# EllarBooher/Syzygy

Hardware: AMD Instinct MI355X
Metric: Mpixels/s deferred-lit+atmosphere (higher is better)
Workload: dtype f32

## Files before the change

### syzygy_amd/csrc/api_skyview.cpp

```cpp

#include <new>

#include "api_common.hpp"
#include "lut_state.hpp"

using namespace szg;

struct szg_skyview
{
    int device = 0;
    szg_skyview_desc desc{};
    DeviceBuffer<float> d_transmittance, d_skyview, d_multiscatter, d_aerialLuminance, d_aerialTransmittance;
    float aerialMaxDistance = 0.0f;
    mutable LutState luts;
    DeviceBuffer<unsigned> d_slutStatusAll;
    bool lutReuse = false;
    DeviceBuffer<unsigned> d_lutKey;
    DeviceBuffer<void> d_framePrep;
    DeviceBuffer<void> d_framePrepDraw;
};

static hipError_t ensure_tlut_status(szg_skyview* p, hipStream_t s)
{
    hipError_t e = hipSuccess;
// ... 89 lines not shown
    }
    return SZG_OK;
}

void szg_skyview_destroy(szg_skyview_t* p)
{
    if (p == nullptr)
    {
        return;
    }
    (void)hipSetDevice(p->device);
    delete p;
}

int szg_skyview_transmittance_lut(const szg_skyview_t* p, szg_image* out)
{
    if (p == nullptr || out == nullptr)
    {
        return fail(SZG_ERR_INVALID_ARGUMENT, "szg_skyview_transmittance_lut: NULL argument");
    }
    *out = make_image(p->d_transmittance, p->desc.transmittance_width, p->desc.transmittance_height, SZG_FORMAT_RGBA32_SFLOAT);
    p->luts.transmittance_exposed();
    return SZG_OK;
}

int szg_skyview_skyview_lut(const szg_skyview_t* p, szg_image* out)
{
    if (p == nullptr || out == nullptr)
    {
        return fail(SZG_ERR_INVALID_ARGUMENT, "szg_skyview_skyview_lut: NULL argument");
    }
    *out = make_image(p->d_skyview, p->desc.skyview_width, p->desc.skyview_height, SZG_FORMAT_RGBA32_SFLOAT);
    p->luts.skyview_exposed();
    return SZG_OK;
}

int szg_skyview_record_transmittance(szg_skyview_t* p, void* stream, uint32_t atmosphere_index,
                                     const szg_atmosphere_packed* d_atmospheres)
{
    if (p == nullptr || d_atmospheres == nullptr)
    {
        return fail(SZG_ERR_INVALID_ARGUMENT, "szg_skyview_record_transmittance: NULL argument");
    }
    DeviceGuard const guard(p->device);
    hipStream_t const s = static_cast<hipStream_t>(stream);
    const unsigned* dirty = nullptr;
    if (p->lutReuse)
    {
        SZG_HIP(szg::launch_lut_key(s, d_atmospheres, atmosphere_index, nullptr, 0u, p->d_lutKey, 0u, p->luts.forceTransmittance,
                                    p->d_transmittance, p->desc.transmittance_width, p->desc.transmittance_height));
        dirty = p->d_lutKey + 69;
    }
    SZG_HIP(szg::launch_transmittance(s, d_atmospheres, atmosphere_index, p->d_transmittance, p->desc.transmittance_width,
                                      p->desc.transmittance_height, dirty));
    p->luts.transmittance_recorded();
    return SZG_OK;
}

int szg_skyview_record_skyview_lut_rows(szg_skyview_t* p, void* stream, uint32_t atmosphere_index,
                                        const szg_atmosphere_packed* d_atmospheres, uint32_t view_camera_index,
                                        const szg_camera_packed* d_cameras, uint32_t row_begin, uint32_t row_end)
{
    if (p == nullptr || d_atmospheres == nullptr || d_cameras == nullptr)
    {
        return fail(SZG_ERR_INVALID_ARGUMENT, "szg_skyview_record_skyview_lut_rows: NULL argument");
    }
    if (row_begin > row_end || row_end > p->desc.skyview_height)
    {
        return fail(SZG_ERR_INVALID_ARGUMENT, "szg_skyview_record_skyview_lut_rows: rows [%u, %u) outside the %u-row LUT", row_begin,
                    row_end, p->desc.skyview_height);
    }
    DeviceGuard const guard(p->device);
    hipStream_t const s = static_cast<hipStream_t>(stream);
    bool const whole = LutState::whole(row_begin, row_end, p->desc.skyview_height);
    SZG_HIP(ensure_tlut_status(p, s));
    const unsigned* dirty = nullptr;
    if (p->lutReuse && whole)
    {
        SZG_HIP(szg::launch_lut_key(s, d_atmospheres, atmosphere_index, d_cameras, view_camera_index, p->d_lutKey, 1u, p->luts.forceSkyview,
                                    p->d_skyview, p->desc.skyview_width, p->desc.skyview_height));
        dirty = p->d_lutKey + 70;
    }
    SZG_HIP(szg::launch_frame_prep(s, d_atmospheres, atmosphere_index, p->desc.transmittance_width, p->desc.transmittance_height,
                                   p->d_framePrep));
    SZG_HIP(szg::launch_skyview(s, d_atmospheres, atmosphere_index, d_cameras, view_camera_index, p->d_transmittance,
                                p->desc.transmittance_width, p->desc.transmittance_height, p->d_skyview, p->desc.skyview_width,
                                p->desc.skyview_height, row_begin, row_end, dirty, p->d_framePrep));
    p->luts.skyview_rows_recorded(row_begin, row_end, p->desc.skyview_height);
    return SZG_OK;
}

int szg_skyview_lut_row_slice(const szg_skyview_t* p, uint32_t rank, uint32_t nranks, uint32_t* row_begin, uint32_t* row_end)
{
    if (p == nullptr || row_begin == nullptr || row_end == nullptr || nranks == 0u || rank >= nranks)
    {
        return fail(SZG_ERR_INVALID_ARGUMENT, "szg_skyview_lut_row_slice: NULL argument or rank outside [0, nranks)");
    }
    if (p->desc.skyview_height % nranks != 0u)
    {
        return fail(SZG_ERR_INVALID_ARGUMENT, "szg_skyview_lut_row_slice: %u LUT rows do not divide over %u ranks", p->desc.skyview_height,
                    nranks);
    }
    uint32_t const n = p->desc.skyview_height / nranks;
    *row_begin = rank * n;
    *row_end = (rank + 1u) * n;
    return SZG_OK;
}

int szg_skyview_allgather_lut_rows(szg_skyview_t* p, szg_rowtile_comm_t* comm, void* stream)
{
    if (p == nullptr || comm == nullptr)
    {
        return fail(SZG_ERR_INVALID_ARGUMENT, "szg_skyview_allgather_lut_rows: NULL argument");
    }
    int const nranks = szg_rowtile_comm_size(comm);
    if (nranks < 1 || p->desc.skyview_height % (uint32_t)nranks != 0u)
    {
        return fail(SZG_ERR_INVALID_ARGUMENT, "szg_skyview_allgather_lut_rows: %u LUT rows do not divide over %d ranks",
                    p->desc.skyview_height, nranks);
    }
    if (nranks > (int)szg::SLUT_STATUS_RANKS)
    {
        return fail(SZG_ERR_INVALID_ARGUMENT, "szg_skyview_allgather_lut_rows: more than %u ranks", szg::SLUT_STATUS_RANKS);
    }
    DeviceGuard const guard(p->device);
    hipStream_t const s = static_cast<hipStream_t>(stream);
    size_t const slice = (size_t)(p->desc.skyview_height / (uint32_t)nranks) * p->desc.skyview_width * 16u;
    unsigned const rank = (unsigned)szg_rowtile_comm_rank(comm);
    bool const known = p->luts.slice_status_known(rank, (uint32_t)nranks, p->desc.skyview_height);
    SZG_HIP(szg::launch_slut_status_stage(s, p->d_slutStatusAll, rank, p->d_skyview, p->desc.skyview_width,
                                          p->desc.skyview_height, known));
    int rc = szg_rowtile_allgather(comm, stream, p->d_skyview, slice);
    if (rc == SZG_OK)
    {
        rc = szg_rowtile_allgather(comm, stream, p->d_slutStatusAll, sizeof(unsigned));
    }
    if (rc == SZG_OK)
    {
        SZG_HIP(szg::launch_slut_status_reduce(s, p->d_slutStatusAll, (unsigned)nranks, p->d_skyview, p->desc.skyview_width,
                                               p->desc.skyview_height));
    }
    p->luts.rows_gathered(rc == SZG_OK);
    return rc;
}

int szg_skyview_record_skyview_lut(szg_skyview_t* p, void* stream, uint32_t atmosphere_index,
                                   const szg_atmosphere_packed* d_atmospheres, uint32_t view_camera_index,
                                   const szg_camera_packed* d_cameras)
{
    if (p == nullptr)
    {
        return fail(SZG_ERR_INVALID_ARGUMENT, "szg_skyview_record_skyview_lut: NULL argument");
    }
    return szg_skyview_record_skyview_lut_rows(p, stream, atmosphere_index, d_atmospheres, view_camera_index, d_cameras, 0u,
                                               p->desc.skyview_height);
}

static int record_composite(szg_skyview_t* p, void* stream, const szg_scene_texture* scene_texture, szg_rect draw_rect,
                            const szg_rowtile* tile, const szg_gbuffer* gbuffer, const szg_shadowmaps* shadow_maps,
                            uint32_t atmosphere_index, const szg_atmosphere_packed* d_atmospheres, uint32_t view_camera_index,
                            const szg_camera_packed* d_cameras, uint32_t sun_light_index,
                            const szg_directional_light_packed* d_lights, bool fast)
{
    if (p == nullptr || d_atmospheres == nullptr || d_cameras == nullptr || d_lights == nullptr)
    {
        return fail(SZG_ERR_INVALID_ARGUMENT, "szg_skyview_record_composite: NULL argument");
    }
    if (!check_rect(draw_rect, "szg_skyview_record_composite"))
    {
        return SZG_ERR_INVALID_ARGUMENT;
    }
    DeviceGuard const guard(p->device);
    if (draw_rect.width == 0u || draw_rect.height == 0u)
    {
        return SZG_OK;
    }
    szg::TileArgs t{};
    if (!resolve_tile(tile, draw_rect.height, t))
    {
        return SZG_ERR_INVALID_ARGUMENT;
    }
    if (!check_scene(scene_texture, draw_rect.width, t.local_rows, true) || !check_gbuffer(gbuffer, draw_rect.width, t.local_rows))
    {
        return SZG_ERR_INVALID_ARGUMENT;
    }
    szg::ShadowSlot sun{nullptr, 0u, 0u, 0u, 0u};
    if (shadow_maps != nullptr && shadow_maps->maps != nullptr && sun_light_index < shadow_maps->count &&
        shadow_maps->maps[sun_light_index].data != nullptr)
    {
        const szg_image& m = shadow_maps->maps[sun_light_index];
        if (!check_image(m, SZG_FORMAT_D32_SFLOAT, 1u, 1u, "shadow map"))
        {
            return SZG_ERR_INVALID_ARGUMENT;
        }
        sun = szg::ShadowSlot{static_cast<const float*>(m.data), m.width, m.height, m.pitch_bytes / 4u, 0u};
    }
    szg::AerialLut aerial{nullptr, SZG_AERIAL_W, SZG_AERIAL_H, SZG_AERIAL_D, 0.0f};
    if (fast)
    {
        if (!(p->aerialMaxDistance > 0.0f))
        {
            return fail(SZG_ERR_INVALID_ARGUMENT, "szg_skyview_record_composite_fast: no aerial LUT has been recorded");
        }
        aerial.luminance = p->d_aerialLuminance;
        aerial.maxDistance = p->aerialMaxDistance;
    }
    SZG_HIP(ensure_tlut_status(p, static_cast<hipStream_t>(stream)));
    SZG_HIP(ensure_slut_status(p, static_cast<hipStream_t>(stream)));
    SZG_HIP(szg::launch_frame_prep(static_cast<hipStream_t>(stream), d_atmospheres, atmosphere_index, p->desc.transmittance_width,
                                   p->desc.transmittance_height, p->d_framePrepDraw,
                                   sun.map != nullptr ? d_lights + sun_light_index : nullptr));
    SZG_HIP(szg::launch_composite(static_cast<hipStream_t>(stream), *scene_texture, draw_rect.width, draw_rect.height, t, *gbuffer,
                                  sun, d_atmospheres, atmosphere_index, d_cameras, view_camera_index, d_lights, sun_light_index,
                                  p->d_transmittance, p->desc.transmittance_width, p->desc.transmittance_height, p->d_skyview,
                                  p->desc.skyview_width, p->desc.skyview_height, aerial, p->d_framePrepDraw));
    return SZG_OK;
}

int szg_skyview_record_composite(szg_skyview_t* p, void* stream, const szg_scene_texture* scene_texture, szg_rect draw_rect,
                                 const szg_rowtile* tile, const szg_gbuffer* gbuffer, const szg_shadowmaps* shadow_maps,
                                 uint32_t atmosphere_index, const szg_atmosphere_packed* d_atmospheres,
                                 uint32_t view_camera_index, const szg_camera_packed* d_cameras, uint32_t sun_light_index,
                                 const szg_directional_light_packed* d_lights)
{
    return record_composite(p, stream, scene_texture, draw_rect, tile, gbuffer, shadow_maps, atmosphere_index, d_atmospheres,
                            view_camera_index, d_cameras, sun_light_index, d_lights, false);
}

int szg_skyview_record_composite_fast(szg_skyview_t* p, void* stream, const szg_scene_texture* scene_texture, szg_rect draw_rect,
                                      const szg_rowtile* tile, const szg_gbuffer* gbuffer, const szg_shadowmaps* shadow_maps,
                                      uint32_t atmosphere_index, const szg_atmosphere_packed* d_atmospheres,
                                      uint32_t view_camera_index, const szg_camera_packed* d_cameras, uint32_t sun_light_index,
                                      const szg_directional_light_packed* d_lights)
{
    return record_composite(p, stream, scene_texture, draw_rect, tile, gbuffer, shadow_maps, atmosphere_index, d_atmospheres,
                            view_camera_index, d_cameras, sun_light_index, d_lights, true);
}

int szg_skyview_record_multiscatter_lut(szg_skyview_t* p, void* stream, uint32_t atmosphere_index,
                                        const szg_atmosphere_packed* d_atmospheres)
{
    if (p == nullptr || d_atmospheres == nullptr)
    {
        return fail(SZG_ERR_INVALID_ARGUMENT, "szg_skyview_record_multiscatter_lut: NULL argument");
    }
    DeviceGuard const guard(p->device);
    SZG_HIP(ensure_tlut_status(p, static_cast<hipStream_t>(stream)));
    SZG_HIP(szg::launch_multiscatter(static_cast<hipStream_t>(stream), d_atmospheres, atmosphere_index, p->d_transmittance,
                                     p->desc.transmittance_width, p->desc.transmittance_height, p->d_multiscatter,
                                     SZG_MULTISCATTER_DIM));
    return SZG_OK;
}

int szg_skyview_multiscatter_lut(const szg_skyview_t* p, szg_image* out)
{
    if (p == nullptr || out == nullptr)
    {
        return fail(SZG_ERR_INVALID_ARGUMENT, "szg_skyview_multiscatter_lut: NULL argument");
    }
    *out = make_image(p->d_multiscatter, SZG_MULTISCATTER_DIM, SZG_MULTISCATTER_DIM, SZG_FORMAT_RGBA32_SFLOAT);
    return SZG_OK;
}

int szg_skyview_record_aerial_lut(szg_skyview_t* p, void* stream, uint32_t atmosphere_index,
                                  const szg_atmosphere_packed* d_atmospheres, uint32_t view_camera_index,
                                  const szg_camera_packed* d_cameras, float max_distance_mm)
{
    if (p == nullptr || d_atmospheres == nullptr || d_cameras == nullptr)
    {
        return fail(SZG_ERR_INVALID_ARGUMENT, "szg_skyview_record_aerial_lut: NULL argument");
    }
    if (!(max_distance_mm > 0.0f) || !(max_distance_mm < 1.0e6f))
    {
        return fail(SZG_ERR_INVALID_ARGUMENT, "szg_skyview_record_aerial_lut: max_distance_mm must be in (0, 1e6)");
    }
    DeviceGuard const guard(p->device);
    SZG_HIP(ensure_tlut_status(p, static_cast<hipStream_t>(stream)));
    SZG_HIP(szg::launch_aerial_lut(static_cast<hipStream_t>(stream), d_atmospheres, atmosphere_index, d_cameras, view_camera_index,
                                   p->d_transmittance, p->desc.transmittance_width, p->desc.transmittance_height,
                                   p->d_aerialLuminance, p->d_aerialTransmittance, SZG_AERIAL_W, SZG_AERIAL_H, SZG_AERIAL_D,
                                   max_distance_mm));
    p->aerialMaxDistance = max_distance_mm;
    return SZG_OK;
}

int szg_skyview_aerial_lut(const szg_skyview_t* p, szg_image* out_luminance, szg_image* out_transmittance)
{
    if (p == nullptr || out_luminance == nullptr || out_transmittance == nullptr)
    {
        return fail(SZG_ERR_INVALID_ARGUMENT, "szg_skyview_aerial_lut: NULL argument");
    }
    *out_luminance = make_image(p->d_aerialLuminance, SZG_AERIAL_W, SZG_AERIAL_H * SZG_AERIAL_D, SZG_FORMAT_RGBA32_SFLOAT);
    *out_transmittance = make_image(p->d_aerialTransmittance, SZG_AERIAL_W, SZG_AERIAL_H * SZG_AERIAL_D, SZG_FORMAT_RGBA32_SFLOAT);
    return SZG_OK;
// ... 16 lines not shown
```

### syzygy_amd/csrc/kernels_lut.hip

```cpp

#include "szg_device.hpp"
#include "szg_launch.hpp"

namespace szg
{
template <int CTRL> SZG_DEV float dpp(float v)
{
    return __builtin_bit_cast(float, __builtin_amdgcn_update_dpp(0, __builtin_bit_cast(int, v), CTRL, 0xF, 0xF, false));
}

constexpr int T_LANES = 8;
constexpr int T_STEPS = 500;

template <bool LEAN> SZG_DEV V3 transmittanceProduct(const Atm& a, V3 origin, V3 direction, float distance, float ndt, int sub)
{
    V3 T = splat(1.0f);
    float const rcp500 = rcpN(500.0f);
#pragma unroll 1
    for (int k = 0; k < (T_STEPS + T_LANES - 1) / T_LANES; k++)
    {
        int const i = k * T_LANES + sub;
        float const t = divRX<LEAN>(distance * ((float)i + 0.5f), 500.0f, rcp500);
        V3 const position = origin + t * direction;
        float const altitude = sqrtPX<LEAN>(dotT(position, position)) - a.planetRadius;
        Extinction const e = sampleExtinction<LEAN>(a, altitude);
        bool const valid = i < T_STEPS;
        float const fx = valid ? expX<LEAN>(ndt * e.extinction.x) : 1.0f;
        float const fy = valid ? expX<LEAN>(ndt * e.extinction.y) : 1.0f;
        float const fz = valid ? expX<LEAN>(ndt * e.extinction.z) : 1.0f;
        T.x = dpp<0x107>(T.x) * fx;
        T.y = dpp<0x107>(T.y) * fy;
        T.z = dpp<0x107>(T.z) * fz;
#pragma unroll
        for (int j = 1; j < T_LANES; j++)
        {
            T.x = dpp<0x111>(T.x) * fx;
            T.y = dpp<0x111>(T.y) * fy;
            T.z = dpp<0x111>(T.z) * fz;
        }
    }
    return T;
}

__global__ __launch_bounds__(256) void k_transmittance(const szg_atmosphere_packed* __restrict__ atmospheres,
                                                      unsigned atmosphereIndex, float4* __restrict__ lut, int W, int H,
                                                      const unsigned* __restrict__ dirty)
{
    if (dirty != nullptr && dirty[0] == 0u)
    {
        return;
    }
    int const sub = (int)(threadIdx.x & (unsigned)(T_LANES - 1));
    int const idRaw = (int)((blockIdx.x * 256u + threadIdx.x) / (unsigned)T_LANES);
    bool const inRangeTexel = idRaw < W * H;
    int const id = inRangeTexel ? idRaw : (W * H - 1);
    int const tx = id % W;
    int const ty = id / W;
    Atm const a = load_atm(atmospheres + atmosphereIndex);

    float const u = ((float)tx + 0.5f) / (float)W;
    float const v = ((float)ty + 0.5f) / (float)H;

    float const x_mu = (u - 0.5f / (float)W) / (1.0f - 1.0f / (float)W);
    float const x_radius = (v - 0.5f / (float)H) / (1.0f - 1.0f / (float)H);
    float const rho = a.H * x_radius;
    float const radius = sqrtf(rho * rho + a.Rp2);
    float const d_min = a.atmosphereRadius - radius;
    float const d_max = rho + a.H;
    float const d = (d_max - d_min) * x_mu + d_min;
    float mu = 1.0f;
    if (d != 0.0f)
    {
        mu = clampf((a.H * a.H - rho * rho - d * d) / (2.0f * radius * d), -1.0f, 1.0f);
    }

    V3 const origin = mk3(0.0f, radius, 0.0f);
    V3 const direction = mk3(sqrtf(1.0f - mu * mu), mu, 0.0f);

    float t0 = 0.0f, t1 = 0.0f;
    bool const hit = raySphere(origin, direction, a.atmosphereRadius, t0, t1);
    float const distance = hit ? t1 : 0.0f;
    float const dt = distance / 500.0f;
    float const ndt = -fabsf(dt);
    float const rmin2 = mu < 0.0f ? radius * radius * (1.0f - mu * mu) : radius * radius;
    bool const lean = waveAll(a.lean && rmin2 >= a.leanFloor2 && inRange(radius, 0x1p-30f, 0x1p30f) && inRange(distance, 0.0f, 0x1p30f));
    V3 const T = lean ? transmittanceProduct<true>(a, origin, direction, distance, ndt, sub)
                      : transmittanceProduct<false>(a, origin, direction, distance, ndt, sub);
    if (inRangeTexel && sub == T_LANES - 1)
    {
        float4 const texel = hit ? make_float4(T.x, T.y, T.z, 1.0f) : make_float4(1.0f, 1.0f, 1.0f, 1.0f);
        lut[id] = texel;
        if (!tlutTexelModerate(texel.x, texel.y, texel.z))
        {
            atomicOr(reinterpret_cast<unsigned*>(lut + (size_t)W * (size_t)H), 1u);
        }
    }
}

__global__ __launch_bounds__(256) void k_lut_range(float4* __restrict__ lut, unsigned n)
{
    unsigned const id = blockIdx.x * 256u + threadIdx.x;
    bool ok = true;
    if (id < n)
    {
        float4 const t = lut[id];
        ok = tlutTexelModerate(t.x, t.y, t.z);
    }
    if (!waveAll(ok) && (threadIdx.x & 63u) == 0u)
    {
        atomicOr(reinterpret_cast<unsigned*>(lut + n), 1u);
    }
}

__global__ __launch_bounds__(64) void k_frame_prep(const szg_atmosphere_packed* __restrict__ atmospheres, unsigned atmosphereIndex,
                                                   int tW, int tH, FramePrep* __restrict__ out,
                                                   const szg_directional_light_packed* __restrict__ sun)
{
    if (threadIdx.x != 0u)
    {
        return;
    }
    FramePrep f;
    f.a = load_atm(atmospheres + atmosphereIndex);
    f.fwidth = (float)tW;
    f.fheight = (float)tH;
    f.u_bias = 0.5f / (float)tW;
    f.u_scale = 1.0f - 1.0f / (float)tW;
    f.v_bias = 0.5f / (float)tH;
    f.v_scale = 1.0f - 1.0f / (float)tH;
    {
        auto vOf = [&](float x_radius) {
            float const t = SZG_CON(SZG_C_LUTMAP, x_radius, f.v_scale, f.v_bias);
            return SZG_CON(SZG_C_TEXCOORD, t, f.fheight, -0.5f);
        };
        float const rMax = sqrtf(f.a.innerCeil2) * (1.0f + 0x1p-16f);
        float const rhoMax = safeSqrt(rMax * rMax - f.a.Rp2);
        float const vLo = vOf(0.0f), vHi = vOf(rhoMax / f.a.H);
        bool const ok = f.a.lean && vLo >= 0.0f && floorf(vHi) + 1.0f <= f.fheight - 1.0f && vHi == vHi && tW >= 2 && tH >= 2 &&
                        (float)tW * (float)tH <= 0x1p24f;
        f.rowsInterior = ok ? 1u : 0u;
    }
#pragma unroll
    for (int k = 0; k < 16; k++)
    {
        f.sunShadow[k] = 0.0f;
    }
    if (sun != nullptr)
    {
        M4 toTex;
        float const t[16] = {0.5f, 0.0f, 0.0f, 0.0f, 0.0f, 0.5f, 0.0f, 0.0f, 0.0f, 0.0f, 1.0f, 0.0f, 0.5f, 0.5f, 0.0f, 1.0f};
#pragma unroll
        for (int k = 0; k < 16; k++)
        {
            toTex.m[k] = t[k];
        }
        M4 const sm = mul(toTex, mul(load_m4(sun->projection), load_m4(sun->view)));
#pragma unroll
        for (int k = 0; k < 16; k++)
        {
            f.sunShadow[k] = sm.m[k];
        }
    }
    *out = f;
}

__global__ __launch_bounds__(256, 4) void k_skyview(const szg_atmosphere_packed* __restrict__ atmospheres, unsigned atmosphereIndex,
                                                 const szg_camera_packed* __restrict__ cameras, unsigned cameraIndex,
                                                 const float4* __restrict__ tlut, int tW, int tH, float4* __restrict__ lut,
                                                 int W, int H, int rowBegin, int rowEnd, const unsigned* __restrict__ dirty,
                                                 const FramePrep* __restrict__ prep)
{
    if (dirty != nullptr && dirty[0] == 0u)
    {
        return;
    }
    unsigned const tid = threadIdx.x;
    unsigned const wave = tid >> 6, lane = tid & 63u;
    int const x = (int)(blockIdx.x * 32u + wave * 8u + (lane & 7u));
    int const y = rowBegin + (int)(blockIdx.y * 8u + (lane >> 3));
    if (x >= W || y >= rowEnd)
    {
        return;
    }
    Atm const a = load_atm(*prep);
    TLut const L = make_tlut(tlut, tW, tH, *prep);
    const szg_camera_packed* cam = cameras + cameraIndex;
    float const PI = 3.141592653589793f;

    float const u = ((float)x + 0.5f) / (float)W;
    float const v = ((float)y + 0.5f) / (float)H;

    V3 origin = mk3(cam->position[0], cam->position[1], cam->position[2]) / 1000000.0f;
    origin.y *= -1.0f;
    origin.y += a.planetRadius;

    float const radius = length(origin);
    float const sinHorizonZenith = a.planetRadius / radius;
    float const horizonZenith = PI - szg_asinf(sinHorizonZenith);
    float const cosineViewLightProjected = (u - 0.5f) * 2.0f;
    V2 const lightDirectionProjected = normalize(V2{-a.incidentDirectionSun.x, -a.incidentDirectionSun.z});
    float azimuthSun = szg_asinf(lightDirectionProjected.x);
    if (lightDirectionProjected.y < 0.0f)
    {
        azimuthSun = PI - azimuthSun;
    }
    float const azimuth = szg_acosf(clampf(cosineViewLightProjected, -1.0f, 1.0f)) + azimuthSun;
    float viewZenith;
    float const unnormalized_v = 2.0f * v - 1.0f;
    if (v < 0.5f)
    {
        float const angleFraction = 1.0f - unnormalized_v * unnormalized_v;
        viewZenith = angleFraction * horizonZenith;
    }
    else
    {
        float const angleFraction = unnormalized_v * unnormalized_v;
        viewZenith = (PI - horizonZenith) * angleFraction + horizonZenith;
    }
    float const elevation = -(viewZenith - PI / 2.0f);

    float const ce = szg_cosf(elevation);
    V3 const direction = normalize(mk3(szg_sinf(azimuth) * ce, szg_sinf(elevation), szg_cosf(azimuth) * ce));

    float const distance = raycastAtmosphere(a, origin, direction);
    V3 const luminance = scatteringIntegral(L, a, origin, direction, distance);
    lut[y * W + x] = make_float4(luminance.x, luminance.y, luminance.z, 1.0f);
    if (!slutTexelFinite(luminance.x, luminance.y, luminance.z))
    {
        atomicOr(reinterpret_cast<unsigned*>(lut + (size_t)W * (size_t)H), 1u);
    }
}

__global__ __launch_bounds__(256) void k_slut_check(float4* __restrict__ lut, unsigned n)
{
    unsigned const id = blockIdx.x * 256u + threadIdx.x;
    bool ok = true;
    if (id < n)
    {
        float4 const t = lut[id];
        ok = slutTexelFinite(t.x, t.y, t.z);
    }
    if (!waveAll(ok) && (threadIdx.x & 63u) == 0u)
    {
        atomicOr(reinterpret_cast<unsigned*>(lut + n), 1u);
    }
}

__global__ void k_slut_status_stage(unsigned* __restrict__ all, unsigned rank, const unsigned* __restrict__ status, unsigned known)
{
    if (threadIdx.x == 0u)
    {
        all[rank] = known != 0u ? status[0] : 1u;
    }
}
__global__ void k_slut_status_reduce(const unsigned* __restrict__ all, unsigned nranks, unsigned* __restrict__ status)
{
    if (threadIdx.x == 0u)
    {
        unsigned v = 0u;
        for (unsigned r = 0; r < nranks; r++)
        {
            v |= all[r];
        }
        status[0] = v;
    }
}

__global__ __launch_bounds__(256) void k_aerial_lut(const szg_atmosphere_packed* __restrict__ atmospheres, unsigned atmosphereIndex,
                                                    const szg_camera_packed* __restrict__ cameras, unsigned cameraIndex,
                                                    const float4* __restrict__ tlut, int tW, int tH, float4* __restrict__ luminance,
                                                    float4* __restrict__ transmittance, unsigned W, unsigned H, unsigned D,
                                                    float maxDistance)
{
    unsigned const id = blockIdx.x * 256u + threadIdx.x;
    if (id >= W * H * D)
    {
        return;
    }
    unsigned const i = id % W, j = (id / W) % H, k = id / (W * H);
    Atm const a = load_atm(atmospheres + atmosphereIndex);
    TLut const L = make_tlut(tlut, tW, tH);
    const szg_camera_packed* cam = cameras + cameraIndex;

    V3 position = mk3(cam->position[0], cam->position[1], cam->position[2]) / 1000000.0f;
    position.y *= -1.0f;
    position.y += a.planetRadius;
    float const clipx = (((float)i + 0.5f) / (float)W - 0.5f) * 2.0f;
    float const clipy = (((float)j + 0.5f) / (float)H - 0.5f) * 2.0f;
// ... 107 lines not shown
}

hipError_t launch_transmittance(hipStream_t s, const szg_atmosphere_packed* d_atm, unsigned atmIndex, float* lut, unsigned W,
                                unsigned H, const unsigned* d_dirty)
{
    unsigned const n = W * H * (unsigned)T_LANES;
    if (d_dirty == nullptr)
    {
        hipError_t const e = hipMemsetAsync(lut + (size_t)W * H * 4u, 0, 4u, s);
        if (e != hipSuccess)
        {
            return e;
        }
    }
    hipLaunchKernelGGL(k_transmittance, dim3((n + 255u) / 256u), dim3(256), 0, s, d_atm, atmIndex, reinterpret_cast<float4*>(lut),
                       (int)W, (int)H, d_dirty);
    return hipGetLastError();
}

__global__ __launch_bounds__(64) void k_lut_key(const szg_atmosphere_packed* __restrict__ atmospheres, unsigned atmosphereIndex,
                                                const szg_camera_packed* __restrict__ cameras, unsigned cameraIndex,
                                                unsigned* __restrict__ state, unsigned which, unsigned force,
                                                unsigned* __restrict__ statusDword)
{
    unsigned const lane = threadIdx.x;
    const unsigned* const atm = reinterpret_cast<const unsigned*>(atmospheres + atmosphereIndex);
    unsigned* const key = state + (which == 0u ? 0u : 32u);
    bool differs = false;
    unsigned mine = 0u;
    if (lane < 32u)
    {
        mine = atm[lane];
        differs = mine != key[lane];
    }
    else if (which == 1u && lane < 35u)
    {
        mine = reinterpret_cast<const unsigned*>((cameras + cameraIndex)->position)[lane - 32u];
        differs = mine != state[64u + (lane - 32u)];
    }
    bool dirty = force != 0u || __builtin_amdgcn_ballot_w64(differs) != 0ull;
    if (which == 1u)
    {
        dirty = dirty || state[67] != state[68];
    }
    if (dirty)
    {
        if (lane < 32u)
        {
            key[lane] = mine;
        }
        else if (which == 1u && lane < 35u)
        {
            state[64u + (lane - 32u)] = mine;
        }
    }
    if (lane == 0u)
    {
        if (dirty)
        {
            if (which == 0u)
            {
                state[67] = state[67] + 1u;
            }
            else
            {
                state[68] = state[67];
            }
            statusDword[0] = 0u;
        }
        state[69u + which] = dirty ? 1u : 0u;
    }
}

hipError_t launch_lut_key(hipStream_t s, const szg_atmosphere_packed* d_atm, unsigned atmIndex, const szg_camera_packed* d_cam,
                          unsigned camIndex, unsigned* d_state, unsigned which, bool force, float* lutBlock, unsigned W, unsigned H)
{
    hipLaunchKernelGGL(k_lut_key, dim3(1), dim3(64), 0, s, d_atm, atmIndex, d_cam, camIndex, d_state, which, force ? 1u : 0u,
                       reinterpret_cast<unsigned*>(lutBlock + (size_t)W * H * 4u));
    return hipGetLastError();
}

size_t frame_prep_bytes() { return sizeof(FramePrep); }
hipError_t launch_frame_prep(hipStream_t s, const szg_atmosphere_packed* d_atm, unsigned atmIndex, unsigned tW, unsigned tH, void* d_prep,
                             const szg_directional_light_packed* d_sun)
{
    hipLaunchKernelGGL(k_frame_prep, dim3(1), dim3(64), 0, s, d_atm, atmIndex, (int)tW, (int)tH, static_cast<FramePrep*>(d_prep), d_sun);
    return hipGetLastError();
}

hipError_t launch_lut_range(hipStream_t s, float* lut, unsigned W, unsigned H)
{
    unsigned const n = W * H;
    hipError_t const e = hipMemsetAsync(lut + (size_t)n * 4u, 0, 4u, s);
    if (e != hipSuccess)
    {
        return e;
    }
    hipLaunchKernelGGL(k_lut_range, dim3((n + 255u) / 256u), dim3(256), 0, s, reinterpret_cast<float4*>(lut), n);
    return hipGetLastError();
}

hipError_t launch_slut_check(hipStream_t s, float* lut, unsigned W, unsigned H)
{
    unsigned const n = W * H;
    hipError_t const e = hipMemsetAsync(lut + (size_t)n * 4u, 0, 4, s);
    if (e != hipSuccess)
    {
        return e;
    }
    hipLaunchKernelGGL(k_slut_check, dim3((n + 255u) / 256u), dim3(256), 0, s, reinterpret_cast<float4*>(lut), n);
    return hipGetLastError();
}

hipError_t launch_slut_status_stage(hipStream_t s, unsigned* d_all, unsigned rank, const float* lut, unsigned W, unsigned H, bool known)
{
    hipLaunchKernelGGL(k_slut_status_stage, dim3(1), dim3(64), 0, s, d_all, rank,
                       reinterpret_cast<const unsigned*>(lut + (size_t)W * H * 4u), known ? 1u : 0u);
    return hipGetLastError();
}
hipError_t launch_slut_status_reduce(hipStream_t s, const unsigned* d_all, unsigned nranks, float* lut, unsigned W, unsigned H)
{
    hipLaunchKernelGGL(k_slut_status_reduce, dim3(1), dim3(64), 0, s, d_all, nranks, reinterpret_cast<unsigned*>(lut + (size_t)W * H * 4u));
    return hipGetLastError();
}

hipError_t launch_skyview(hipStream_t s, const szg_atmosphere_packed* d_atm, unsigned atmIndex, const szg_camera_packed* d_cam,
                          unsigned camIndex, const float* tlut, unsigned tW, unsigned tH, float* lut, unsigned W, unsigned H,
                          unsigned rowBegin, unsigned rowEnd, const unsigned* d_dirty, const void* d_prep)
{
    if (rowEnd > H)
    {
        rowEnd = H;
    }
    if (rowBegin >= rowEnd || W == 0u)
    {
        return hipSuccess;
    }
    if (d_dirty == nullptr)
    {
        hipError_t const e = hipMemsetAsync(lut + (size_t)W * H * 4u, 0, 4, s);
        if (e != hipSuccess)
        {
            return e;
        }
    }
    dim3 const grid((W + 31u) / 32u, (rowEnd - rowBegin + 7u) / 8u);
    hipLaunchKernelGGL(k_skyview, grid, dim3(256), 0, s, d_atm, atmIndex, d_cam, camIndex, reinterpret_cast<const float4*>(tlut),
                       (int)tW, (int)tH, reinterpret_cast<float4*>(lut), (int)W, (int)H, (int)rowBegin, (int)rowEnd, d_dirty,
                       static_cast<const FramePrep*>(d_prep));
    return hipGetLastError();
}
}
```

### syzygy_amd/csrc/szg_device.hpp

```cpp
#pragma once

#include <hip/hip_fp16.h>
#include <hip/hip_runtime.h>

#include "szg/abi.h"
#include "szg/fpmath.h"

#define SZG_DEV __device__ __forceinline__

namespace szg
{
struct V2
{
    float x, y;
};
struct V3
{
    float x, y, z;
};
struct V4
{
    float x, y, z, w;
};

// ... 458 lines not shown

SZG_DEV bool raySphere(V3 f, V3 d, float radius, float& t0, float& t1)
{
    float const b = -1.0f * dotA(f, d);
    V3 const chord = f + b * d;
    float const discriminant = radius * radius - dotA(chord, chord);
    float const c = dotA(f, f) - radius * radius;
    if (discriminant < 0.0f)
    {
        return false;
    }
    float q = b;
    float const s = sqrtf(discriminant);
    q = (b < 0.0f) ? (q - s) : (q + s);
    float a0 = c / q;
    float a1 = q;
    if (a0 > a1)
    {
        float const tmp = a0;
        a0 = a1;
        a1 = tmp;
    }
    t0 = a0;
    t1 = a1;
    return true;
}

SZG_DEV float raycastAtmosphere(const Atm& a, V3 origin, V3 direction)
{
    float at0 = 0.0f, at1 = 0.0f;
    bool const hitAtmosphere = raySphere(origin, direction, a.atmosphereRadius, at0, at1) && at1 > 0.0f;
    at0 = fmaxf(0.0f, at0);
    float pt0 = 0.0f, pt1 = 0.0f;
    bool const hitPlanet = raySphere(origin, direction, a.planetRadius, pt0, pt1) && pt0 > 0.0f;
    if (hitPlanet)
    {
        at1 = fminf(pt0, at1);
    }
    return hitAtmosphere ? (at1 - at0) : 0.0f;
}

struct TLut
{
    const float4* texels;
    int width, height;
    float fwidth, fheight;
    float u_bias, u_scale, v_bias, v_scale;
    bool moderate;
    bool rowsInterior;
#ifdef SZG_EXP_LDS_TLUT
    const __attribute__((address_space(3))) float* ldsRows;
#endif
};
SZG_DEV bool tlutTexelModerate(float x, float y, float z)
{
    return inRange(x, 0x1p-50f, 2.0f) && inRange(y, 0x1p-50f, 2.0f) && inRange(z, 0x1p-50f, 2.0f);
}
SZG_DEV TLut make_tlut(const float4* texels, int w, int h)
{
    TLut t;
    t.moderate = reinterpret_cast<const unsigned*>(texels + (size_t)w * (size_t)h)[0] == 0u;
    t.texels = texels;
    t.width = w;
    t.height = h;
    t.fwidth = (float)w;
    t.fheight = (float)h;
    t.u_bias = 0.5f / (float)w;
    t.u_scale = 1.0f - 1.0f / (float)w;
    t.v_bias = 0.5f / (float)h;
    t.v_scale = 1.0f - 1.0f / (float)h;
    t.rowsInterior = false;
#ifdef SZG_EXP_LDS_TLUT
    t.ldsRows = nullptr;
#endif
    return t;
}

struct FramePrep
{
    Atm a;
    float fwidth, fheight, u_bias, u_scale, v_bias, v_scale;
    float sunShadow[16];
    unsigned rowsInterior;
};
SZG_DEV float inVector(float x)
{
    asm volatile("" : "+v"(x));
    return x;
}
SZG_DEV V3 inVector(V3 v) { return V3{inVector(v.x), inVector(v.y), inVector(v.z)}; }
SZG_DEV Atm load_atm(const FramePrep& f)
{
    Atm a = f.a;
    a.scatteringRayleigh = inVector(a.scatteringRayleigh);
    a.densityScaleRayleigh = inVector(a.densityScaleRayleigh);
    a.absorptionRayleigh = inVector(a.absorptionRayleigh);
    a.planetRadius = inVector(a.planetRadius);
    a.scatteringMie = inVector(a.scatteringMie);
    a.densityScaleMie = inVector(a.densityScaleMie);
    a.atmosphereRadius = inVector(a.atmosphereRadius);
    a.incidentDirectionSun = inVector(a.incidentDirectionSun);
    a.scatteringOzone = inVector(a.scatteringOzone);
    a.absorptionOzone = inVector(a.absorptionOzone);
    a.sunIntensitySpectrum = inVector(a.sunIntensitySpectrum);
    a.sunAngularRadius = inVector(a.sunAngularRadius);
    a.Ra2 = inVector(a.Ra2);
    a.Rp2 = inVector(a.Rp2);
    a.H = inVector(a.H);
    a.rcpH = inVector(a.rcpH);
    a.rcpDsR = inVector(a.rcpDsR);
    a.rcpDsM = inVector(a.rcpDsM);
    a.rcp15 = inVector(a.rcp15);
    a.leanFloor2 = inVector(a.leanFloor2);
    a.extFloor2 = inVector(a.extFloor2);
    a.extCeil2 = inVector(a.extCeil2);
    a.innerCeil2 = inVector(a.innerCeil2);
    return a;
}
SZG_DEV TLut make_tlut(const float4* texels, int w, int h, const FramePrep& f)
{
    TLut t;
    t.moderate = reinterpret_cast<const unsigned*>(texels + (size_t)w * (size_t)h)[0] == 0u;
    t.texels = texels;
    t.width = w;
    t.height = h;
    t.fwidth = inVector(f.fwidth);
    t.fheight = inVector(f.fheight);
    t.u_bias = inVector(f.u_bias);
    t.u_scale = inVector(f.u_scale);
    t.v_bias = inVector(f.v_bias);
    t.v_scale = inVector(f.v_scale);
    t.rowsInterior = f.rowsInterior != 0u;
#ifdef SZG_EXP_LDS_TLUT
    t.ldsRows = nullptr;
#endif
    return t;
}

SZG_DEV V3 bilinear_rgb(const float4* __restrict__ texels, int W, int H, float fW, float fH, float s, float t)
{
    float const u = SZG_CON(SZG_C_TEXCOORD, s, fW, -0.5f);
    float const v = SZG_CON(SZG_C_TEXCOORD, t, fH, -0.5f);
    float const fu = floorf(u);
    float const fv = floorf(v);
    float const a = u - fu;
    float const b = v - fv;
    int i0 = (int)fu, j0 = (int)fv;
    int i1 = i0 + 1, j1 = j0 + 1;
    i0 = min(max(i0, 0), W - 1);
    i1 = min(max(i1, 0), W - 1);
    j0 = min(max(j0, 0), H - 1);
    j1 = min(max(j1, 0), H - 1);
    float4 const t00 = texels[j0 * W + i0];
    float4 const t10 = texels[j0 * W + i1];
    float4 const t01 = texels[j1 * W + i0];
    float4 const t11 = texels[j1 * W + i1];
    float const w00 = (1.0f - a) * (1.0f - b);
    float const w10 = a * (1.0f - b);
    float const w01 = (1.0f - a) * b;
    float const w11 = a * b;
    V3 r;
    r.x = SZG_CON(SZG_C_BILINEAR, w11, t11.x, SZG_CON(SZG_C_BILINEAR, w01, t01.x, SZG_CON(SZG_C_BILINEAR, w10, t10.x, w00 * t00.x)));
    r.y = SZG_CON(SZG_C_BILINEAR, w11, t11.y, SZG_CON(SZG_C_BILINEAR, w01, t01.y, SZG_CON(SZG_C_BILINEAR, w10, t10.y, w00 * t00.y)));
    r.z = SZG_CON(SZG_C_BILINEAR, w11, t11.z, SZG_CON(SZG_C_BILINEAR, w01, t01.z, SZG_CON(SZG_C_BILINEAR, w10, t10.z, w00 * t00.z)));
    return r;
}
// ... 442 lines not shown
```

### syzygy_amd/csrc/szg_launch.hpp

```cpp
#pragma once

#include <hip/hip_runtime_api.h>

#include "szg/abi.h"
#include "szg/compute_collection.h"
#include "szg/debuglines.h"
#include "szg/present.h"
#include "szg/raster.h"
#include "szg/texture_display.h"
#include "szg/ui_layer.h"

namespace szg
{
struct LightRec
{
    float shadowRows[16];
    float dir[3];
    float falloffFactor;
    float colorStrength[3];
    float falloffDistance;
    float position[3];
    unsigned isSpot;
    const float* map;
    unsigned mapWidth, mapHeight;
    unsigned mapPitchFloats;
    unsigned leanOK;
    float falloffBound;
    float rcpFalloffDistance;
};
static_assert(sizeof(LightRec) == 144, "LightRec layout");

struct ShadowSlot
{
    const float* map;
    unsigned width, height, pitchFloats, pad;
};
static_assert(sizeof(ShadowSlot) == 24, "ShadowSlot layout");

struct AerialLut
{
    const float* luminance;
    unsigned W, H, D;
    float maxDistance;
};

struct TileArgs
{
    unsigned block_rows, rank, nranks, local_rows;
};

inline size_t tlut_block_bytes(unsigned W, unsigned H) { return (size_t)W * H * 16u + 16u; }
hipError_t launch_lut_range(hipStream_t s, float* lut, unsigned W, unsigned H);
hipError_t launch_transmittance(hipStream_t s, const szg_atmosphere_packed* d_atm, unsigned atmIndex, float* lut, unsigned W,
                                unsigned H, const unsigned* d_dirty = nullptr);
constexpr unsigned LUT_KEY_DWORDS = 72u;
constexpr unsigned SLUT_STATUS_RANKS = 64u;
hipError_t launch_lut_key(hipStream_t s, const szg_atmosphere_packed* d_atm, unsigned atmIndex, const szg_camera_packed* d_cam,
                          unsigned camIndex, unsigned* d_state, unsigned which, bool force, float* lutBlock, unsigned W, unsigned H);
inline size_t slut_block_bytes(unsigned W, unsigned H) { return (size_t)W * H * 16u + 16u; }
hipError_t launch_slut_check(hipStream_t s, float* lut, unsigned W, unsigned H);
hipError_t launch_slut_status_stage(hipStream_t s, unsigned* d_all, unsigned rank, const float* lut, unsigned W, unsigned H, bool known);
hipError_t launch_slut_status_reduce(hipStream_t s, const unsigned* d_all, unsigned nranks, float* lut, unsigned W, unsigned H);
hipError_t launch_skyview(hipStream_t s, const szg_atmosphere_packed* d_atm, unsigned atmIndex, const szg_camera_packed* d_cam,
                          unsigned camIndex, const float* tlut, unsigned tW, unsigned tH, float* lut, unsigned W, unsigned H,
                          unsigned rowBegin, unsigned rowEnd, const unsigned* d_dirty, const void* d_prep);
size_t frame_prep_bytes();
hipError_t launch_frame_prep(hipStream_t s, const szg_atmosphere_packed* d_atm, unsigned atmIndex, unsigned tW, unsigned tH, void* d_prep,
                             const szg_directional_light_packed* d_sun = nullptr);
hipError_t launch_light_prep(hipStream_t s, const szg_directional_light_packed* d_dir, unsigned dirCount, unsigned dirSkip,
                             const szg_spot_light_packed* d_spot, unsigned spotCount, const ShadowSlot* d_slots,
                             unsigned slotCount, LightRec* d_out);
hipError_t launch_lights(hipStream_t s, const szg_scene_texture& scene, unsigned drawW, unsigned drawH, TileArgs tile,
                         const szg_gbuffer& g, const szg_camera_packed* d_cam, unsigned camIndex, const LightRec* d_lights,
                         unsigned lightCount, const unsigned long long* d_tileMasks);
hipError_t launch_light_tiles(hipStream_t s, unsigned drawW, unsigned drawH, TileArgs tile, const szg_gbuffer& g,
                              const LightRec* d_lights, unsigned lightCount, unsigned long long* d_tileMasks);
hipError_t launch_gbuffer_fill(hipStream_t s, const szg_scene_texture& scene, unsigned drawW, unsigned drawH, TileArgs tile,
                               const szg_gbuffer& g, const szg_camera_packed* d_cam, unsigned camIndex, float ground_y,
                               float ground_half_extent, float checker_cell, float ground_roughness,
                               const szg_fill_box* d_boxes, unsigned boxCount);
hipError_t launch_composite(hipStream_t s, const szg_scene_texture& scene, unsigned drawW, unsigned drawH, TileArgs tile,
                            const szg_gbuffer& g, ShadowSlot sunSlot, const szg_atmosphere_packed* d_atm, unsigned atmIndex, const szg_camera_packed* d_cam,
                            unsigned camIndex, const szg_directional_light_packed* d_dir, unsigned sunIndex, const float* tlut,
                            unsigned tW, unsigned tH, const float* slut, unsigned sW, unsigned sH, AerialLut aerial, const void* d_prep);
hipError_t launch_aerial_lut(hipStream_t s, const szg_atmosphere_packed* d_atm, unsigned atmIndex, const szg_camera_packed* d_cam,
                             unsigned camIndex, const float* tlut, unsigned tW, unsigned tH, float* luminance, float* transmittance,
                             unsigned W, unsigned H, unsigned D, float maxDistance);
hipError_t launch_multiscatter(hipStream_t s, const szg_atmosphere_packed* d_atm, unsigned atmIndex, const float* tlut, unsigned tW,
                               unsigned tH, float* out, unsigned dim);
struct ShadowGen
{
    float projView[16];
    float invProjView[16];
    float* map;
    unsigned dim, pitchFloats, pad;
};
hipError_t launch_shadow_maps(hipStream_t s, const szg_directional_light_packed* d_dir, unsigned dirCount,
                              const szg_spot_light_packed* d_spot, unsigned spotCount, const ShadowSlot* d_ownedSlots,
                              unsigned slotCount, ShadowGen* d_gen, const szg_fill_box* d_boxes, unsigned boxCount, unsigned maxDim);
hipError_t launch_shadow_prep(hipStream_t s, const szg_directional_light_packed* d_dir, unsigned dirCount,
                              const szg_spot_light_packed* d_spot, unsigned spotCount, const ShadowSlot* d_ownedSlots,
                              unsigned slotCount, ShadowGen* d_gen);

struct alignas(128) RasterDraw
{
    const szg_vertex_packed* vertices;
    const uint32_t* indices;
    const szg_mat4* models;
    const szg_mat4* mits;
    uint32_t vertexCount, firstIndex, triCount, instanceCount;
    uint32_t firstPrim;
    uint32_t pad;
    szg_texture tex[3];
    const void* mipChain[3];
    uint32_t mipLevels[3];
    float maxLod;
};
static_assert(sizeof(RasterDraw) == 256, "RasterDraw layout");
struct PrimRec
{
    float a[3], b[3], c[3];
    float z[3], w[3];
    uint32_t draw, instance, tri;
    float hx[3], hy[3], noise[3];
    float facing;
};
static_assert(sizeof(PrimRec) == 112, "PrimRec layout");
struct RasterBuffers
{
    PrimRec* prims = nullptr;
    uint2* boxes = nullptr;
    unsigned* keysA = nullptr;
    unsigned* keysB = nullptr;
    unsigned* valsA = nullptr;
    unsigned* valsB = nullptr;
    uint2* orderedBoxes = nullptr;
    uint2* chunkBoxes = nullptr;
    uint2* superBoxes = nullptr;
    void* sortTemp = nullptr;
    size_t sortTempBytes = 0;
    const unsigned* order = nullptr;
    size_t capacity = 0;
};
constexpr unsigned RASTER_SORT_THRESHOLD = 4096u;
hipError_t raster_sort_temp_bytes(unsigned n, size_t& bytes);
hipError_t raster_sort_pairs(hipStream_t s, void* temp, size_t tempBytes, const unsigned* keysIn, unsigned* keysOut,
                             const unsigned* valsIn, unsigned* valsOut, unsigned n);
hipError_t launch_raster_setup(hipStream_t s, bool shadow, const RasterDraw* d_draws, unsigned drawCount, unsigned primCount,
                               const szg_camera_packed* d_cam, unsigned camIndex, const ShadowGen* d_gen, unsigned W, unsigned H,
                               RasterBuffers& b);
hipError_t launch_raster_tile(hipStream_t s, const szg_scene_texture& scene, unsigned drawW, unsigned drawH, TileArgs tile,
// ... 92 lines not shown
```

Baseline: 2581.

## Hoist skyview camera setup into frame prep and fold status clear into prep kernel

Moves the per-pixel camera origin, horizon zenith and sun azimuth computation from the skyview kernel into the single-thread frame-prep kernel, which now also zeroes the skyview status word instead of a separate hipMemsetAsync. The transmittance product now evaluates two consecutive steps per lane per round, halving the number of DPP shift chains. The aim is to cut redundant per-thread math, one memset enqueue and serial DPP latency, at the cost of more live registers per round and a larger FramePrep struct.

```diff
diff --git a/syzygy_amd/csrc/api_skyview.cpp b/syzygy_amd/csrc/api_skyview.cpp
--- a/syzygy_amd/csrc/api_skyview.cpp
+++ b/syzygy_amd/csrc/api_skyview.cpp
@@ -195,7 +195,9 @@
         dirty = p->d_lutKey + 70;
     }
     SZG_HIP(szg::launch_frame_prep(s, d_atmospheres, atmosphere_index, p->desc.transmittance_width, p->desc.transmittance_height,
-                                   p->d_framePrep));
+                                   p->d_framePrep, nullptr, d_cameras, view_camera_index,
+                                   szg::skyview_status_to_clear(p->d_skyview, p->desc.skyview_width, p->desc.skyview_height, row_begin,
+                                                                row_end, dirty)));
     SZG_HIP(szg::launch_skyview(s, d_atmospheres, atmosphere_index, d_cameras, view_camera_index, p->d_transmittance,
                                 p->desc.transmittance_width, p->desc.transmittance_height, p->d_skyview, p->desc.skyview_width,
                                 p->desc.skyview_height, row_begin, row_end, dirty, p->d_framePrep));
@@ -322,7 +324,7 @@
     SZG_HIP(ensure_slut_status(p, static_cast<hipStream_t>(stream)));
     SZG_HIP(szg::launch_frame_prep(static_cast<hipStream_t>(stream), d_atmospheres, atmosphere_index, p->desc.transmittance_width,
                                    p->desc.transmittance_height, p->d_framePrepDraw,
-                                   sun.map != nullptr ? d_lights + sun_light_index : nullptr));
+                                   sun.map != nullptr ? d_lights + sun_light_index : nullptr, d_cameras, view_camera_index));
     SZG_HIP(szg::launch_composite(static_cast<hipStream_t>(stream), *scene_texture, draw_rect.width, draw_rect.height, t, *gbuffer,
                                   sun, d_atmospheres, atmosphere_index, d_cameras, view_camera_index, d_lights, sun_light_index,
                                   p->d_transmittance, p->desc.transmittance_width, p->desc.transmittance_height, p->d_skyview,
diff --git a/syzygy_amd/csrc/kernels_lut.hip b/syzygy_amd/csrc/kernels_lut.hip
--- a/syzygy_amd/csrc/kernels_lut.hip
+++ b/syzygy_amd/csrc/kernels_lut.hip
@@ -1,6 +1,7 @@
 
 #include "szg_device.hpp"
 #include "szg_launch.hpp"
+#include "szg_tchain.hpp"
 
 namespace szg
 {
@@ -9,34 +10,39 @@
     return __builtin_bit_cast(float, __builtin_amdgcn_update_dpp(0, __builtin_bit_cast(int, v), CTRL, 0xF, 0xF, false));
 }
 
-constexpr int T_LANES = 8;
-constexpr int T_STEPS = 500;
-
+template <bool LEAN> SZG_DEV V3 transmittanceFactor(const Atm& a, V3 origin, V3 direction, float distance, float ndt, float rcp500, int i)
+{
+    float const t = divRX<LEAN>(distance * ((float)i + 0.5f), 500.0f, rcp500);
+    V3 const position = origin + t * direction;
+    float const altitude = sqrtPX<LEAN>(dotT(position, position)) - a.planetRadius;
+    Extinction const e = sampleExtinction<LEAN>(a, altitude);
+    bool const valid = tchainValid(i);
+    V3 f;
+    f.x = valid ? expX<LEAN>(ndt * e.extinction.x) : 1.0f;
+    f.y = valid ? expX<LEAN>(ndt * e.extinction.y) : 1.0f;
+    f.z = valid ? expX<LEAN>(ndt * e.extinction.z) : 1.0f;
+    return f;
+}
+
+static_assert(T_PER_LANE == 2, "transmittanceProduct multiplies two factors per lane and round");
 template <bool LEAN> SZG_DEV V3 transmittanceProduct(const Atm& a, V3 origin, V3 direction, float distance, float ndt, int sub)
 {
     V3 T = splat(1.0f);
     float const rcp500 = rcpN(500.0f);
 #pragma unroll 1
-    for (int k = 0; k < (T_STEPS + T_LANES - 1) / T_LANES; k++)
-    {
-        int const i = k * T_LANES + sub;
-        float const t = divRX<LEAN>(distance * ((float)i + 0.5f), 500.0f, rcp500);
-        V3 const position = origin + t * direction;
-        float const altitude = sqrtPX<LEAN>(dotT(position, position)) - a.planetRadius;
-        Extinction const e = sampleExtinction<LEAN>(a, altitude);
-        bool const valid = i < T_STEPS;
-        float const fx = valid ? expX<LEAN>(ndt * e.extinction.x) : 1.0f;
-        float const fy = valid ? expX<LEAN>(ndt * e.extinction.y) : 1.0f;
-        float const fz = valid ? expX<LEAN>(ndt * e.extinction.z) : 1.0f;
-        T.x = dpp<0x107>(T.x) * fx;
-        T.y = dpp<0x107>(T.y) * fy;
-        T.z = dpp<0x107>(T.z) * fz;
+    for (int k = 0; k < T_ROUNDS; k++)
+    {
+        V3 const f0 = transmittanceFactor<LEAN>(a, origin, direction, distance, ndt, rcp500, tchainStep(T_LANES, k, sub, 0));
+        V3 const f1 = transmittanceFactor<LEAN>(a, origin, direction, distance, ndt, rcp500, tchainStep(T_LANES, k, sub, 1));
+        T.x = dpp<0x107>(T.x) * f0.x * f1.x;
+        T.y = dpp<0x107>(T.y) * f0.y * f1.y;
+        T.z = dpp<0x107>(T.z) * f0.z * f1.z;
 #pragma unroll
         for (int j = 1; j < T_LANES; j++)
         {
-            T.x = dpp<0x111>(T.x) * fx;
-            T.y = dpp<0x111>(T.y) * fy;
-            T.z = dpp<0x111>(T.z) * fz;
+            T.x = dpp<0x111>(T.x) * f0.x * f1.x;
+            T.y = dpp<0x111>(T.y) * f0.y * f1.y;
+            T.z = dpp<0x111>(T.z) * f0.z * f1.z;
         }
     }
     return T;
@@ -114,11 +120,17 @@
 
 __global__ __launch_bounds__(64) void k_frame_prep(const szg_atmosphere_packed* __restrict__ atmospheres, unsigned atmosphereIndex,
                                                    int tW, int tH, FramePrep* __restrict__ out,
-                                                   const szg_directional_light_packed* __restrict__ sun)
+                                                   const szg_directional_light_packed* __restrict__ sun,
+                                                   const szg_camera_packed* __restrict__ cameras, unsigned cameraIndex,
+                                                   unsigned* __restrict__ clearStatus)
 {
     if (threadIdx.x != 0u)
     {
         return;
+    }
+    if (clearStatus != nullptr)
+    {
+        clearStatus[0] = 0u;
     }
     FramePrep f;
     f.a = load_atm(atmospheres + atmosphereIndex);
@@ -161,6 +173,28 @@
             f.sunShadow[k] = sm.m[k];
         }
     }
+    f.skyOrigin = splat(0.0f);
+    f.skyHorizonZenith = 0.0f;
+    f.skyAzimuthSun = 0.0f;
+    if (cameras != nullptr)
+    {
+        const szg_camera_packed* cam = cameras + cameraIndex;
+        float const PI = 3.141592653589793f;
+        V3 origin = mk3(cam->position[0], cam->position[1], cam->position[2]) / 1000000.0f;
+        origin.y *= -1.0f;
+        origin.y += f.a.planetRadius;
+        float const radius = length(origin);
+        float const sinHorizonZenith = f.a.planetRadius / radius;
+        V2 const lightDirectionProjected = normalize(V2{-f.a.incidentDirectionSun.x, -f.a.incidentDirectionSun.z});
+        float azimuthSun = szg_asinf(lightDirectionProjected.x);
+        if (lightDirectionProjected.y < 0.0f)
+        {
+            azimuthSun = PI - azimuthSun;
+        }
+        f.skyOrigin = origin;
+        f.skyHorizonZenith = PI - szg_asinf(sinHorizonZenith);
+        f.skyAzimuthSun = azimuthSun;
+    }
     *out = f;
 }
 
@@ -184,26 +218,15 @@
     }
     Atm const a = load_atm(*prep);
     TLut const L = make_tlut(tlut, tW, tH, *prep);
-    const szg_camera_packed* cam = cameras + cameraIndex;
     float const PI = 3.141592653589793f;
 
     float const u = ((float)x + 0.5f) / (float)W;
     float const v = ((float)y + 0.5f) / (float)H;
 
-    V3 origin = mk3(cam->position[0], cam->position[1], cam->position[2]) / 1000000.0f;
-    origin.y *= -1.0f;
-    origin.y += a.planetRadius;
-
-    float const radius = length(origin);
-    float const sinHorizonZenith = a.planetRadius / radius;
-    float const horizonZenith = PI - szg_asinf(sinHorizonZenith);
+    V3 const origin = inVector(prep->skyOrigin);
+    float const horizonZenith = prep->skyHorizonZenith;
+    float const azimuthSun = prep->skyAzimuthSun;
     float const cosineViewLightProjected = (u - 0.5f) * 2.0f;
-    V2 const lightDirectionProjected = normalize(V2{-a.incidentDirectionSun.x, -a.incidentDirectionSun.z});
-    float azimuthSun = szg_asinf(lightDirectionProjected.x);
-    if (lightDirectionProjected.y < 0.0f)
-    {
-        azimuthSun = PI - azimuthSun;
-    }
     float const azimuth = szg_acosf(clampf(cosineViewLightProjected, -1.0f, 1.0f)) + azimuthSun;
     float viewZenith;
     float const unnormalized_v = 2.0f * v - 1.0f;
@@ -477,9 +500,11 @@
 
 size_t frame_prep_bytes() { return sizeof(FramePrep); }
 hipError_t launch_frame_prep(hipStream_t s, const szg_atmosphere_packed* d_atm, unsigned atmIndex, unsigned tW, unsigned tH, void* d_prep,
-                             const szg_directional_light_packed* d_sun)
-{
-    hipLaunchKernelGGL(k_frame_prep, dim3(1), dim3(64), 0, s, d_atm, atmIndex, (int)tW, (int)tH, static_cast<FramePrep*>(d_prep), d_sun);
+                             const szg_directional_light_packed* d_sun, const szg_camera_packed* d_cam, unsigned camIndex,
+                             unsigned* d_clearStatus)
+{
+    hipLaunchKernelGGL(k_frame_prep, dim3(1), dim3(64), 0, s, d_atm, atmIndex, (int)tW, (int)tH, static_cast<FramePrep*>(d_prep), d_sun,
+                       d_cam, camIndex, d_clearStatus);
     return hipGetLastError();
 }
 
@@ -530,14 +555,6 @@
     if (rowBegin >= rowEnd || W == 0u)
     {
         return hipSuccess;
-    }
-    if (d_dirty == nullptr)
-    {
-        hipError_t const e = hipMemsetAsync(lut + (size_t)W * H * 4u, 0, 4, s);
-        if (e != hipSuccess)
-        {
-            return e;
-        }
     }
     dim3 const grid((W + 31u) / 32u, (rowEnd - rowBegin + 7u) / 8u);
     hipLaunchKernelGGL(k_skyview, grid, dim3(256), 0, s, d_atm, atmIndex, d_cam, camIndex, reinterpret_cast<const float4*>(tlut),
diff --git a/syzygy_amd/csrc/szg_device.hpp b/syzygy_amd/csrc/szg_device.hpp
--- a/syzygy_amd/csrc/szg_device.hpp
+++ b/syzygy_amd/csrc/szg_device.hpp
@@ -564,6 +564,8 @@
     float fwidth, fheight, u_bias, u_scale, v_bias, v_scale;
     float sunShadow[16];
     unsigned rowsInterior;
+    V3 skyOrigin;
+    float skyHorizonZenith, skyAzimuthSun;
 };
 SZG_DEV float inVector(float x)
 {
diff --git a/syzygy_amd/csrc/szg_launch.hpp b/syzygy_amd/csrc/szg_launch.hpp
--- a/syzygy_amd/csrc/szg_launch.hpp
+++ b/syzygy_amd/csrc/szg_launch.hpp
@@ -66,7 +66,13 @@
                           unsigned rowBegin, unsigned rowEnd, const unsigned* d_dirty, const void* d_prep);
 size_t frame_prep_bytes();
 hipError_t launch_frame_prep(hipStream_t s, const szg_atmosphere_packed* d_atm, unsigned atmIndex, unsigned tW, unsigned tH, void* d_prep,
-                             const szg_directional_light_packed* d_sun = nullptr);
+                             const szg_directional_light_packed* d_sun = nullptr, const szg_camera_packed* d_cam = nullptr,
+                             unsigned camIndex = 0u, unsigned* d_clearStatus = nullptr);
+inline unsigned* skyview_status_to_clear(float* lut, unsigned W, unsigned H, unsigned rowBegin, unsigned rowEnd, const unsigned* d_dirty)
+{
+    bool const launches = rowBegin < (rowEnd < H ? rowEnd : H) && W != 0u;
+    return (d_dirty == nullptr && launches) ? reinterpret_cast<unsigned*>(lut + (size_t)W * H * 4u) : nullptr;
+}
 hipError_t launch_light_prep(hipStream_t s, const szg_directional_light_packed* d_dir, unsigned dirCount, unsigned dirSkip,
                              const szg_spot_light_packed* d_spot, unsigned spotCount, const ShadowSlot* d_slots,
                              unsigned slotCount, LightRec* d_out);
diff --git a/syzygy_amd/csrc/szg_tchain.hpp b/syzygy_amd/csrc/szg_tchain.hpp
--- /dev/null
+++ b/syzygy_amd/csrc/szg_tchain.hpp
@@ -0,0 +1,14 @@
+#pragma once
+
+namespace szg
+{
+constexpr int T_STEPS = 500;
+constexpr int T_LANES = 8;
+constexpr int T_PER_LANE = 2;
+
+constexpr int tchainRounds(int lanes) { return (T_STEPS + lanes * T_PER_LANE - 1) / (lanes * T_PER_LANE); }
+constexpr int tchainStep(int lanes, int k, int sub, int j) { return (k * lanes + sub) * T_PER_LANE + j; }
+constexpr bool tchainValid(int step) { return step < T_STEPS; }
+
+constexpr int T_ROUNDS = tchainRounds(T_LANES);
+}
```

After: 2586, median of 6. About the same (+0.2%).
